# chongminggao/CIRS-codes

Measured on AMD Instinct MI355X. Metric: simulator env-steps/s (collect + PPO update in the timed region), KuaishouEnv, higher is better.
Workload: dtype f32 (policy/tracker; rollout on the fp32 MFMA, PPO head products fp32-accurate from two fp16 pieces per operand (3 f16 MFMAs per product), fp32 accumulate) + f64 (env rewards, GAE)

## Files before the change

### cirs-codes_amd/csrc/small_gemm.h

```cpp
#pragma once
#include "common.h"

namespace cirs {

typedef float sg_f32x16 __attribute__((ext_vector_type(16)));

template <bool kNT>
__device__ __forceinline__ void rows_gemm_body(int bx, int by, const float* __restrict__ X, int ldx, const float* __restrict__ W, int ldw,
                                               const float* __restrict__ bias, int R, int Kd, int N, int relu,
                                               const float* __restrict__ relu_of, int accumulate, float* __restrict__ Y, int ldy,
                                               const long* __restrict__ out_row) {
    const int lane = threadIdx.x, hi = lane >> 5, lo = lane & 31;
    const int row0 = bx * 32, n0 = by * 32;
    const int row = row0 + lo, n = n0 + lo;
    const bool row_ok = row < R, n_ok = n < N;
    sg_f32x16 acc;
    const float b = (bias && n_ok) ? bias[n] : 0.f;
#pragma unroll
    for (int s = 0; s < 16; ++s) acc[s] = b;
    const float* xr = X + (size_t)(row_ok ? row : 0) * ldx;
    if (kNT && (Kd & 31) == 0 && (ldx & 3) == 0 && ((uintptr_t)X & 15) == 0 && (ldw & 3) == 0 && ((uintptr_t)W & 15) == 0) {
        const float* wr = W + (size_t)(n_ok ? n : 0) * ldw;
        for (int kk = 0; kk < Kd; kk += 32) {
            float a[16], bv[16];
// ... 66 lines not shown
                                    const long* out_row = nullptr) {
    const dim3 grid(cdiv(R, 32), cdiv(N, 32));
    if (nt) hipLaunchKernelGGL(rows_gemm_kernel<true>, grid, dim3(64), 0, s, X, ldx, W, ldw, bias, R, Kd, N, relu, relu_of, accumulate, Y, ldy, out_row);
    else hipLaunchKernelGGL(rows_gemm_kernel<false>, grid, dim3(64), 0, s, X, ldx, W, ldw, bias, R, Kd, N, relu, relu_of, accumulate, Y, ldy, out_row);
}

constexpr int kDwMaxSlabs = 256;
__host__ inline int dwg_slabs(long R) {
    const long want = (R + 63) / 64;
    return (int)(want < 1 ? 1 : (want > kDwMaxSlabs ? kDwMaxSlabs : want));
}
__host__ inline size_t dwg_partial_floats(long R, int O, int K) { return (size_t)dwg_slabs(R) * O * (K + 1); }

__device__ __forceinline__ void dw_gemm_body(int bx, int slab, const float* __restrict__ dY, int ldy, const float* __restrict__ X, int ldx, int R,
                                             int O, int K, int rows_per_slab, float* __restrict__ partial) {
    const int lane = threadIdx.x, hi = lane >> 5, lo = lane & 31;
    const int k_tiles = (K + 31) / 32;
    const int o0 = (bx / k_tiles) * 32, k0 = (bx % k_tiles) * 32;
    const int r_beg = slab * rows_per_slab, r_end = min(R, r_beg + rows_per_slab);
    const int o = o0 + lo, k = k0 + lo;
    const bool o_ok = o < O, k_ok = k < K;
    sg_f32x16 acc;
#pragma unroll
    for (int s = 0; s < 16; ++s) acc[s] = 0.f;
    float bsum = 0.f;
    for (int r = r_beg; r < r_end; r += 64) {
        float a[32], b[32];
#pragma unroll
        for (int j = 0; j < 32; ++j) {
            const int rr = r + 2 * j + hi;
            const bool r_ok = rr < r_end;
// ... 185 lines not shown
```

### cirs-codes_amd/csrc/tracker_bwd.hip

```cpp
#include <algorithm>
#include "tracker_rows.h"
#include "rng.h"

namespace cirs {

#ifdef CIRS_TBWD_PROF
__device__ unsigned long long g_tbwd_prof[64];
#define CIRS_BSTAMP(K) do { if ((int)blockIdx.x == 300 && threadIdx.x == 0) g_tbwd_prof[K] = __builtin_amdgcn_s_memtime(); } while (0)
__device__ unsigned long long g_tbwd_wg[2048 * 3];
#define CIRS_BWG(SEL, WHICH) do { if ((SEL) && threadIdx.x == 0 && blockIdx.x < 2048) { g_tbwd_wg[blockIdx.x * 3 + (WHICH)] = __builtin_amdgcn_s_memtime(); \
    if ((WHICH) == 0) { unsigned hw; asm volatile("s_getreg_b32 %0, hwreg(HW_REG_HW_ID)" : "=s"(hw)); unsigned xcc; asm volatile("s_getreg_b32 %0, hwreg(HW_REG_XCC_ID)" : "=s"(xcc)); g_tbwd_wg[blockIdx.x * 3 + 2] = ((unsigned long long)xcc << 32) | hw; } } } while (0)
#else
#define CIRS_BSTAMP(K) do { } while (0)
#define CIRS_BWG(SEL, WHICH) do { } while (0)
#endif
constexpr int kChunkRows = 256;

struct DropCfg {
    int on;
    uint32_t thr;
    float inv;
    uint64_t seed;
    int env_base;
};
// ... 389 lines not shown
                }
            }
        }
#pragma unroll
        for (int h = 0; h < HPL; ++h) {
            const float ia = (kDrop ? dc.inv : 1.0f) / smA[h], ib = (kDrop ? dc.inv : 1.0f) / smB[h];
#pragma unroll
            for (int d = 0; d < HD; ++d) { accA[h * HD + d] *= ia; accB[h * HD + d] *= ib; }
        }
        if (actA) ep_store(ATT + (size_t)(base + pA) * tD + hg * DPL, accA, 1.0f);
        if (actB) ep_store(ATT + (size_t)(base + pB) * tD + hg * DPL, accB, 1.0f);
    }
}

template <int NH, bool kDrop>
__global__ __launch_bounds__(64) void attn_bwd_ep(const float* __restrict__ QKV, const float* __restrict__ dATT,
                                                  const int32_t* __restrict__ offsets, const int32_t* __restrict__ lens, int Lp,
                                                  float* __restrict__ dQKV, DropCfg dc, int layer,
                                                  const uint32_t* __restrict__ keep_in ) {
    using G = EpGeo<NH>;
    constexpr int HPL = G::HPL, DPL = G::DPL, HD = G::HD, SL = G::SL;
    extern __shared__ __attribute__((aligned(16))) float smem[];
    const int b = blockIdx.x, len = lens[b];
    if (len <= 0) return;
    const int lane = threadIdx.x, hg = lane / SL, slot = lane - hg * SL;
    const int base = offsets[b], STR = G::strip(Lp);
    float* sQKV = smem;
    float* sdA = smem + (size_t)Lp * 96;
    float* sS = sdA + (size_t)Lp * 32;
    float* sM = sS + (size_t)G::NW * (Lp + 1) * STR;
    float* sI = sM + (size_t)NH * Lp;
    uint32_t* sK = reinterpret_cast<uint32_t*>(sI + (size_t)NH * Lp);
    CIRS_BWG(layer == 1, 0);
    CIRS_BSTAMP(39);
    const int len32 = min(len, 32);
    f32x4 st_q[12], st_d[4];
    ep_stage_issue<96, 12>(st_q, QKV + (size_t)base * 96, len32, 96, lane);
    ep_stage_issue<tD, 4>(st_d, dATT + (size_t)base * tD, len32, tD, lane);
// ... 168 lines not shown
                }
            }
        }
        if (actA) {
            float* o = dQKV + (size_t)(base + jA) * 96 + 32 + hg * DPL;
            ep_store(o, dKA, scale); ep_store(o + 32, dVA, 1.0f);
        }
        if (actB) {
            float* o = dQKV + (size_t)(base + jB) * 96 + 32 + hg * DPL;
            ep_store(o, dKB, scale); ep_store(o + 32, dVB, 1.0f);
        }
    }
    CIRS_BSTAMP(42);
    CIRS_BWG(layer == 1, 1);
}
#undef EP_KEEP

constexpr int kRowT = 132;
__device__ __forceinline__ void mm_block(sg_f32x16& acc, const float (&a)[16], const float* __restrict__ wr) {
    float bv[16];
    ep_load(bv, wr);
#pragma unroll
    for (int j = 0; j < 16; ++j) acc = __builtin_amdgcn_mfma_f32_32x32x2f32(a[j], bv[j], acc, 0, 0, 0);
}
__device__ __forceinline__ void acc_to_lds(float* __restrict__ sT, const sg_f32x16& acc, int col, int hi) {
#pragma unroll
    for (int s = 0; s < 16; ++s) sT[acc_row(s, hi) * kRowT + col] = acc[s];
}
__device__ __forceinline__ void ln_half_row(const float (&y)[16], const float* __restrict__ g, const float* __restrict__ b, int hi,
                                            float (&xh)[16], float (&out)[16], float& rs) {
// ... 371 lines not shown
    acc_to_lds(sT, acc, lo, hi);
    __syncthreads();
    {
        float t[16];
        ep_load(t, sT + lo * kRowT + 16 * hi);
        if (row_ok) ep_store(a.dATT + rr * tD + 16 * hi, t, 1.0f);
    }
    CIRS_BSTAMP(28);
}

struct BwdScratch {
    float *G, *H[CIRS_MAX_TRACKER_LAYERS + 1];
    float *QKV[CIRS_MAX_TRACKER_LAYERS], *P[CIRS_MAX_TRACKER_LAYERS], *ATT[CIRS_MAX_TRACKER_LAYERS];
    float *XH1[CIRS_MAX_TRACKER_LAYERS], *RS1[CIRS_MAX_TRACKER_LAYERS], *H1N[CIRS_MAX_TRACKER_LAYERS], *FF1[CIRS_MAX_TRACKER_LAYERS];
    float *XH2[CIRS_MAX_TRACKER_LAYERS], *RS2[CIRS_MAX_TRACKER_LAYERS];
    float *T0, *T1, *T2, *T3, *T4, *T5, *dQKV, *dFF1, *dS, *partial, *GIN;
    float* LC;
    float* PM[CIRS_MAX_TRACKER_LAYERS];
    void* sort;
};

constexpr int kLastFloats = tD + 16 + 2 + 2;

static size_t bwd_partial_floats(const cirs_tracker_cfg* cfg, long R) {
    size_t f = dw_list_floats(R, 32, tD) + dw_list_floats(R, tD, tD) + dw_list_floats(R, tD, tD + 1);
    f += (size_t)cfg->nlayers * (2 * dw_list_floats(R, tD, tD) + dw_list_floats(R, tD, tH) + dw_list_floats(R, tH, tD) +
                                 dw_list_floats(R, tD, tD) + dw_list_floats(R, 96, tD));
    return f;
}

static size_t bwd_floats(const cirs_tracker_cfg* cfg, long R) {
    const long nl = cfg->nlayers, Lp = cfg->max_len, NH = cfg->nhead;
    size_t f = 0;
    f += (size_t)R * 32;
    f += (size_t)(nl + 1) * R * tD;
    f += (size_t)nl * R * (96 + NH * Lp + tD + tD + 1 + tD + tH + tD + 1);
    f += 6 * (size_t)R * tD + (size_t)R * 96 + (size_t)R * tH + (size_t)R * NH * Lp + 64;
    if (cfg->dropout_p > 0.f) f += (size_t)nl * R * NH * Lp + 64;
    f += bwd_partial_floats(cfg, R) + 4096;
    f += (size_t)R * (tD + 1);
    f += (size_t)R * kLastFloats;
    f += emb_sort_bytes(R + cfg->n_env) / 4 + 64;
    return f + 64 * 32;
}

static BwdScratch carve_bwd(void* ws, const cirs_tracker_cfg* cfg, long R) {
    float* p = (float*)ws;
    auto take = [&](size_t n) { float* r = p; p += (n + 3) & ~(size_t)3; return r; };
    const long nl = cfg->nlayers, Lp = cfg->max_len, NH = cfg->nhead;
    BwdScratch s;
    s.G = take((size_t)R * 32);
    for (int l = 0; l <= nl; ++l) s.H[l] = take((size_t)R * tD);
    for (int l = 0; l < nl; ++l) {
        s.QKV[l] = take((size_t)R * 96); s.P[l] = take((size_t)R * NH * Lp); s.ATT[l] = take((size_t)R * tD);
        s.XH1[l] = take((size_t)R * tD); s.RS1[l] = take(R); s.H1N[l] = take((size_t)R * tD); s.FF1[l] = take((size_t)R * tH);
        s.XH2[l] = take((size_t)R * tD); s.RS2[l] = take(R);
    }
    s.T0 = take((size_t)R * tD); s.T1 = take((size_t)R * tD); s.T2 = take((size_t)R * tD); s.T3 = take((size_t)R * tD);
    s.T4 = take((size_t)R * tD); s.T5 = take((size_t)R * tD);
    for (int l = 0; l < nl; ++l) s.PM[l] = cfg->dropout_p > 0.f ? take((size_t)R * NH * Lp) : nullptr;
    s.dQKV = take((size_t)R * 96); s.dFF1 = take((size_t)R * tH); s.dS = take((size_t)R * NH * Lp);
    s.partial = take(bwd_partial_floats(cfg, R) + 4096);
    s.GIN = take((size_t)R * (tD + 1));
    s.LC = take((size_t)R * kLastFloats);
    s.sort = (void*)take(emb_sort_bytes(R + cfg->n_env) / 4 + 64);
    return s;
}

}

#ifdef CIRS_TBWD_PROF
extern "C" int cirs_debug_tbwd_wg(unsigned long long* out_host) {
    return hipMemcpyFromSymbol(out_host, HIP_SYMBOL(cirs::g_tbwd_wg), 2048 * 3 * sizeof(unsigned long long)) == hipSuccess ? 0 : -2;
}
extern "C" int cirs_debug_tbwd_prof(unsigned long long* out_host64) {
    return hipMemcpyFromSymbol(out_host64, HIP_SYMBOL(cirs::g_tbwd_prof), 64 * sizeof(unsigned long long)) == hipSuccess ? 0 : -2;
// ... 617 lines not shown
    const bool ep = L <= 64 && ep_bytes(true) <= 64 * 1024 && !getenv("CIRS_TRACKER_ATTN_ROWS");
#define ATT_EP1(KERNEL, N, BWD, ...)                                                                                            \
    do {                                                                                                                        \
        if (dc.on) CIRS_LAUNCH_SPREAD((KERNEL<N, true>), B, 0, ep_bytes(BWD), s, __VA_ARGS__);       \
        else CIRS_LAUNCH_SPREAD((KERNEL<N, false>), B, 0, ep_bytes(BWD), s, __VA_ARGS__);           \
    } while (0)
#define ATT_EP(KERNEL, BWD, ...)                                  \
    do {                                                          \
        switch (NH) {                                             \
            case 1: ATT_EP1(KERNEL, 1, BWD, __VA_ARGS__); break;  \
            case 2: ATT_EP1(KERNEL, 2, BWD, __VA_ARGS__); break;  \
            case 4: ATT_EP1(KERNEL, 4, BWD, __VA_ARGS__); break;  \
            default: ATT_EP1(KERNEL, 8, BWD, __VA_ARGS__); break; \
        }                                                         \
    } while (0)

    DropCfg dc{};
    if (cfg->dropout_p > 0.f) {
        CIRS_REQUIRE(cfg->dropout_p < 1.f, "dropout_p must be in [0, 1)");
        dc.on = 1; dc.thr = dropout_threshold(cfg->dropout_p); dc.inv = 1.0f / (1.0f - cfg->dropout_p);
        dc.seed = cfg->dropout_seed; dc.env_base = cfg->drop_env_base;
    }
    if (state_out && ep && L <= 32 && S <= 64 && !getenv("CIRS_TRACKER_PREFIX_LAUNCHES")) {
        PrefixEnvArgs pa{};
        pa.x_hist = st->x_hist; pa.pe = w->pe; pa.row_env = row_env; pa.row_t = row_t; pa.offsets = offsets; pa.lens = lens;
        for (int l = 0; l < nl; ++l) pa.layer[l] = w->layer[l];
        pa.dec_w = w->dec_w; pa.dec_b = w->dec_b; pa.state_out = state_out; pa.state_stride = (long)state_stride; pa.nl = nl; pa.L = L; pa.S = S;
        if (ptf && ptf->on) {
            CIRS_REQUIRE(ptf->cfg.hidden == kH && ptf->cfg.dim_state == S && ptf->h2, "prefix states: trunk shape mismatch");
            pa.tf = *ptf;
// ... 64 lines not shown
        }
        LayerFwdArgs fa{sc.ATT[l], sc.H[l], y, l + 1 < nl ? w->layer[l + 1].in_proj_w : nullptr, l + 1 < nl ? w->layer[l + 1].in_proj_b : nullptr,
                        sc.XH1[l], sc.RS1[l], sc.H1N[l], sc.FF1[l], sc.XH2[l], sc.RS2[l], sc.H[l + 1], l + 1 < nl ? sc.QKV[l + 1] : nullptr,
                        row_env, row_t, R, l};
        if (dc.on) CIRS_LAUNCH_SPREAD(layer_rows_fwd<true>, cdiv(R, 32), 40 * 1024, 0, s, fa, dc);
        else CIRS_LAUNCH_SPREAD(layer_rows_fwd<false>, cdiv(R, 32), 40 * 1024, 0, s, fa, dc);
    }
    CIRS_CHECK_LAUNCH("tracker forward recompute");
    if (state_out) {
        hipLaunchKernelGGL(prefix_decoder_kernel, dim3(cdiv(B, 4)), dim3(256), 0, s, (const float*)sc.H[nl], lens, B, S, w->dec_w, w->dec_b,
                           state_out, (long)state_stride);
        CIRS_CHECK_LAUNCH("prefix_decoder_kernel");
        return CIRS_OK;
    }
    float* dH = sc.T0;
    if (top_last) {
        hipLaunchKernelGGL(dstate_last_rows, g1((long)B * S), dim3(256), 0, s, dstate_last, lens, B, S, sc.G);
        launch_rows_gemm(false, sc.G, S, w->dec_w, tD, nullptr, B, S, tD, 0, nullptr, 0, dH, tD, s);
    } else {
        if (dstate_last) hipLaunchKernelGGL(dstate_last_full, g1((long)R * S), dim3(256), 0, s, dstate_last, row_env, offsets, lens, R, S, sc.G);
        else hipLaunchKernelGGL(gather_dstate, g1((long)R * S), dim3(256), 0, s, dstate, row_env, row_t, R, S, B, sc.G);
        launch_rows_gemm_dw(dwl, sc.H[nl], tD, S, tD, grads->dec_w, grads->dec_b, sc.partial, false, sc.G, S, w->dec_w, tD, nullptr, R, S, tD, 0, nullptr, 0,
                            dH, tD, s);
    }
    for (int l = nl - 1; l >= 0; --l) {
        const cirs_tracker_layer& y = w->layer[l];
        const cirs_tracker_layer_grads& gy = grads->layer[l];
        if (top_last && l == nl - 1) {
            float* dB1 = dc.on ? sc.T4 : dY1c;
            LayerBwdArgs ba{sc.T0, nullptr, nullptr, nullptr, sc.T0, 0, y, sc.XH2[l], sc.RS2[l], sc.FF1[l], sc.XH1[l], sc.RS1[l], sc.T3, sc.dFF1, sc.T1, dY1c, dB1,
                            sc.T5, env_c, t_c, B, l};
            if (dc.on) CIRS_LAUNCH_SPREAD(layer_rows_bwd<true>, cdiv(B, 32), 40 * 1024, 0, s, ba, dc);
            else CIRS_LAUNCH_SPREAD(layer_rows_bwd<false>, cdiv(B, 32), 40 * 1024, 0, s, ba, dc);
            DwBatch bt{};
            dw_batch_add(bt, dwl, sc.G, S, sc.H[nl], tD, R, S, tD, grads->dec_w, grads->dec_b, 0, sc.partial);
            dw_batch_add(bt, dwl, sc.T0, tD, sc.XH2[l], tD, R, tD, tD, gy.norm2_w, gy.norm2_b, 1, sc.partial);
            dw_batch_add(bt, dwl, sc.T3, tD, sc.FF1[l], tH, R, tD, tH, gy.lin2_w, gy.lin2_b, 0, sc.partial);
            dw_batch_add(bt, dwl, sc.dFF1, tH, sc.H1N[l], tD, R, tH, tD, gy.lin1_w, gy.lin1_b, 0, sc.partial);
            dw_batch_add(bt, dwl, sc.T1, tD, sc.XH1[l], tD, R, tD, tD, gy.norm1_w, gy.norm1_b, 1, sc.partial);
            dw_batch_add(bt, dwl, dB1, tD, sc.ATT[l], tD, R, tD, tD, gy.out_proj_w, gy.out_proj_b, 0, sc.partial);
            dw_batch_launch(bt, R, s, B);
            ATT_LAST(attn_last_bwd, (const float*)sc.QKV[l], (const float*)sc.T5, (const float*)dY1c, (const float*)att_stats, offsets, lens, B, L, sc.dQKV,
                     sc.T2, dc, l);
            continue;
        }
        const bool pre = l + 1 < nl;
        float* dB1 = dc.on ? sc.T4 : sc.T2;
        LayerBwdArgs ba{sc.T0, pre ? sc.T2 : nullptr, pre ? sc.dQKV : nullptr, pre ? w->layer[l + 1].in_proj_w : nullptr, sc.T0, 0, y,
                        sc.XH2[l], sc.RS2[l], sc.FF1[l], sc.XH1[l], sc.RS1[l], sc.T3, sc.dFF1, sc.T1, sc.T2, dB1, sc.T5, row_env, row_t, R, l};
        if (dc.on) CIRS_LAUNCH_SPREAD(layer_rows_bwd<true>, cdiv(R, 32), 40 * 1024, 0, s, ba, dc);
        else CIRS_LAUNCH_SPREAD(layer_rows_bwd<false>, cdiv(R, 32), 40 * 1024, 0, s, ba, dc);
        DwBatch bt{};
        if (pre) dw_batch_add(bt, dwl, sc.dQKV, 96, sc.H[l + 1], tD, R, 96, tD, grads->layer[l + 1].in_proj_w, grads->layer[l + 1].in_proj_b, 0, sc.partial);
        dw_batch_add(bt, dwl, sc.T0, tD, sc.XH2[l], tD, R, tD, tD, gy.norm2_w, gy.norm2_b, 1, sc.partial);
        dw_batch_add(bt, dwl, sc.T3, tD, sc.FF1[l], tH, R, tD, tH, gy.lin2_w, gy.lin2_b, 0, sc.partial);
        dw_batch_add(bt, dwl, sc.dFF1, tH, sc.H1N[l], tD, R, tH, tD, gy.lin1_w, gy.lin1_b, 0, sc.partial);
        dw_batch_add(bt, dwl, sc.T1, tD, sc.XH1[l], tD, R, tD, tD, gy.norm1_w, gy.norm1_b, 1, sc.partial);
        dw_batch_add(bt, dwl, dB1, tD, sc.ATT[l], tD, R, tD, tD, gy.out_proj_w, gy.out_proj_b, 0, sc.partial);
        dw_batch_launch(bt, R, s);
        const float* dATT = sc.T5;
        if (ep) {
            ATT_EP(attn_bwd_ep, true, (const float*)sc.QKV[l], dATT, offsets, lens, L, sc.dQKV, dc, l, dc.on ? reinterpret_cast<const uint32_t*>(sc.P[l]) : (const uint32_t*)nullptr);
        } else {
            ATT_DISPATCH_SH(attn_bwd_q, (size_t)4 * NH * L * sizeof(float), sc.QKV[l], sc.P[l], dATT, row_env, row_t, offsets, R, L, sc.dS, sc.dQKV,
                            (const float*)sc.PM[l], dc.inv);
            ATT_DISPATCH(attn_bwd_kv, sc.QKV[l], dc.on ? sc.PM[l] : sc.P[l], sc.dS, dATT, row_env, row_t, offsets, lens, R, L, sc.dQKV);
        }
    }
    {
        LayerBwdArgs ba{};
        ba.dY1p = sc.T2; ba.dQKVp = sc.dQKV; ba.winp = w->layer[0].in_proj_w; ba.dHout = sc.T0; ba.only_pre = 1;
        ba.row_env = row_env; ba.row_t = row_t; ba.R = R;
        if (dc.on) CIRS_LAUNCH_SPREAD(layer_rows_bwd<true>, cdiv(R, 32), 40 * 1024, 0, s, ba, dc);
        else CIRS_LAUNCH_SPREAD(layer_rows_bwd<false>, cdiv(R, 32), 40 * 1024, 0, s, ba, dc);
    }
    CIRS_CHECK_LAUNCH("tracker backward layers");
    float* DU = sc.T1;
    float* EU = sc.H[nl];
    float* DPRE = sc.H1N[0];
    float* CU = sc.QKV[0];
    float* CI = sc.QKV[0] + (size_t)R * tD;
    int32_t* key_user = (int32_t*)sc.RS1[0];
    int32_t* key_item = (int32_t*)sc.RS2[0];
    const bool merged = B <= R;
    const int slot_rpw = R >= (1 << 17) ? 8 : 1;
    hipLaunchKernelGGL(slot_bwd, dim3(cdiv(R, 4 * slot_rpw)), dim3(256), 0, s, *w, dH, users, act, rew, row_env, row_t, R, B, DU, EU, DPRE,
                       sc.GIN, CU, CI, key_user, key_item, merged ? CI + (size_t)R * tD : nullptr, slot_rpw, 5.656854249492381f);
    if (merged) {
        if (int rc = emb_scatter_merged(key_item, users, lens, CI, R, B, cfg->n_items, cfg->n_users, grads->emb_item, grads->emb_user, sc.sort,
                                        emb_sort_bytes(R + B), s)) return rc;
    } else {
        int32_t* keys_c = (int32_t*)sc.T0;
        float* contrib_c = sc.T2;
        CIRS_HIP(hipMemsetAsync(keys_c, 0xFF, sizeof(int32_t) * (size_t)B, s));
        hipLaunchKernelGGL(compact_user_rows, dim3(cdiv(R, 8)), dim3(256), 0, s, row_env, row_t, users, (const float*)CU, R, keys_c, contrib_c);
        if (int rc = emb_scatter_sorted(keys_c, contrib_c, B, cfg->n_users, grads->emb_user, sc.sort, emb_sort_bytes(R), s)) return rc;
        if (int rc = emb_scatter_sorted(key_item, CI, R, cfg->n_items, grads->emb_item, sc.sort, emb_sort_bytes(R), s)) return rc;
    }
    DwBatch bt{};
    dw_batch_add(bt, dwl, sc.dQKV, 96, sc.H[0], tD, R, 96, tD, grads->layer[0].in_proj_w, grads->layer[0].in_proj_b, 0, sc.partial);
    dw_batch_add(bt, dwl, DU, tD, EU, tD, R, tD, tD, grads->ffn_user_w, grads->ffn_user_b, 0, sc.partial);
    dw_batch_add(bt, dwl, DPRE, tD, sc.GIN, tD + 1, R, tD, tD + 1, grads->gate_w, grads->gate_b, 0, sc.partial);
    dw_batch_launch(bt, R, s);
    launch_dw_list_final(dwl, R, sc.partial, s);
    CIRS_CHECK_LAUNCH("tracker backward slots");
#undef ATT_LAST
#undef ATT_LAST1
#undef ATT_DISPATCH
#undef ATT_EP
#undef ATT_EP1
#undef ATT_DISPATCH_SH
    return CIRS_OK;
}

extern "C" int cirs_tracker_backward(const cirs_tracker_cfg* cfg, const cirs_tracker_weights* w, const cirs_tracker_state* st,
                                     const int32_t* users, const int64_t* act, const double* rew, const int32_t* row_env,
                                     const int32_t* row_t, const int32_t* offsets, const int32_t* lens, int32_t n_rows,
                                     const float* dstate, const cirs_tracker_grads* grads, void* workspace,
                                     int64_t workspace_bytes, void* stream) {
    CIRS_REQUIRE(users && act && rew && dstate && grads, "null argument");
    return tracker_rows_impl(cfg, w, st, users, act, rew, row_env, row_t, offsets, lens, n_rows, dstate, grads, workspace, workspace_bytes, stream,
                             nullptr, 0);
}
// ... 42 lines not shown
```

### cirs-codes_amd/csrc/tracker_rows.h

```cpp
#pragma once
#include <hipcub/hipcub.hpp>
#include "small_gemm.h"
#include "internal.h"

namespace cirs {
typedef float f32x4 __attribute__((ext_vector_type(4)));

constexpr int tD = 32, tH = 128;

constexpr int kMaxDwBatch = 8;
struct DwBatchJob { const float* dY; int ldy; const float* X; int ldx; int O, K, tile_begin; float* partial; };
struct DwBatch { DwBatchJob j[kMaxDwBatch]; int n, total_tiles; };
static __global__ __launch_bounds__(64) void dw_batch_kernel(DwBatch jobs, int R, int rows_per_slab) {
    int ji = 0;
    for (; ji + 1 < jobs.n && (int)blockIdx.x >= jobs.j[ji + 1].tile_begin; ++ji) {}
    const DwBatchJob& jb = jobs.j[ji];
    dw_gemm_body((int)blockIdx.x - jb.tile_begin, blockIdx.y, jb.dY, jb.ldy, jb.X, jb.ldx, R, jb.O, jb.K, rows_per_slab, jb.partial);
}
static inline void dw_batch_add(DwBatch& b, DwList& list, const float* dY, int ldy, const float* X, int ldx, int R, int O, int K, float* dW,
                                float* db, int diag, float* partial) {
    const int slabs = dwg_slabs(R);
    DwListJob& lj = list.j[list.n++];
    lj.O = O; lj.K = K; lj.part_off = list.part_floats; lj.diag = diag; lj.dW = dW; lj.db = db;
    DwBatchJob& jb = b.j[b.n++];
    jb.dY = dY; jb.ldy = ldy; jb.X = X; jb.ldx = ldx; jb.O = O; jb.K = K; jb.tile_begin = b.total_tiles; jb.partial = partial + lj.part_off;
    b.total_tiles += cdiv(O, 32) * cdiv(K, 32);
    list.part_floats += slabs * O * (K + 1);
    list.total_out += O * (K + 1);
}
static inline void dw_batch_launch(const DwBatch& b, int R, hipStream_t s, int R_rows = -1) {
    if (!b.n) return;
    if (R_rows < 0) R_rows = R;
    const int slabs = dwg_slabs(R);
    int rows_per_slab = (R_rows + slabs - 1) / slabs;
    rows_per_slab = (rows_per_slab + 15) & ~15;
    hipLaunchKernelGGL(dw_batch_kernel, dim3(b.total_tiles, slabs), dim3(64), 0, s, b, R_rows, rows_per_slab);
}

static __global__ __launch_bounds__(256) void gather_dstate(const float* __restrict__ dstate, const int32_t* __restrict__ row_env,
                                                     const int32_t* __restrict__ row_t, int R, int S, int B, float* __restrict__ G) {
    const long i = blockIdx.x * (long)blockDim.x + threadIdx.x;
    if (i >= (long)R * S) return;
    const int r = (int)(i / S), s = (int)(i % S);
    G[i] = dstate[((size_t)row_t[r] * B + row_env[r]) * S + s];
}

__device__ __forceinline__ float lane_bcast(float x, int k) {
    return __builtin_bit_cast(float, __builtin_amdgcn_readlane(__builtin_bit_cast(int, x), k));
}

static __global__ __launch_bounds__(256) void slot_bwd(cirs_tracker_weights w, const float* __restrict__ dH0, const int32_t* __restrict__ users,
// ... 66 lines not shown
    rows[r] = r;
}

static __global__ __launch_bounds__(256) void compact_user_rows(const int32_t* __restrict__ row_env, const int32_t* __restrict__ row_t,
                                                         const int32_t* __restrict__ users, const float* __restrict__ CU, int R,
                                                         int32_t* __restrict__ keys_c, float* __restrict__ contrib_c) {
    const int d = threadIdx.x & 31;
    const int r = blockIdx.x * 8 + (threadIdx.x >> 5);
    if (r >= R || row_t[r] != 0) return;
    const int b = row_env[r];
    contrib_c[(size_t)b * tD + d] = CU[(size_t)r * tD + d];
    if (d == 0) keys_c[b] = users[b];
}

constexpr int kSubRun = 64;
static __global__ __launch_bounds__(256) void emb_subrun_kernel(const uint32_t* __restrict__ ks, const int32_t* __restrict__ rs,
                                                         const float* __restrict__ contrib, int R, int n_table, float* __restrict__ part) {
    const int d = threadIdx.x & 31, half = (threadIdx.x >> 5) & 1;
    const int p = blockIdx.x * 8 + (threadIdx.x >> 5);
    const bool in = p < R;
    const uint32_t key = in ? ks[p] : 0xffffffffu;
    const bool start = in && key < (uint32_t)n_table && ((p % kSubRun) == 0 || ks[p - 1] != key);
    const int end = min(R, (p / kSubRun + 1) * kSubRun);
    const int q0 = p + d, q1 = p + 32 + d;
    const bool s0 = start && q0 < end && ks[q0] == key, s1 = start && q1 < end && ks[q1] == key;
    const int r0 = s0 ? rs[q0] : 0, r1 = s1 ? rs[q1] : 0;
    const unsigned long long m0 = __ballot(s0), m1 = __ballot(s1);
    if (!start) return;
    const uint32_t h0 = (uint32_t)(m0 >> (32 * half)), h1 = (uint32_t)(m1 >> (32 * half));
    const int n = h0 == 0xffffffffu ? 32 + (h1 == 0xffffffffu ? 32 : __builtin_ctz(~h1)) : __builtin_ctz(~h0);
    float acc = 0.f;
    for (int q = 0; q < n; q += 16) {
        float t[16];
#pragma unroll
        for (int u = 0; u < 16; ++u) {
            const int qq = q + u;
            const int row = __shfl(qq < 32 ? r0 : r1, (qq & 31) + 32 * half, CIRS_WAVE);
            t[u] = qq < n ? contrib[(size_t)row * tD + d] : 0.f;
        }
#pragma unroll
        for (int u = 0; u < 16; ++u) acc += (q + u < n) ? t[u] : 0.f;
    }
    part[(size_t)p * tD + d] = acc;
}

static __global__ __launch_bounds__(256) void emb_segment_sum_kernel(const uint32_t* __restrict__ ks, const float* __restrict__ part, int R,
                                                              int n_table, float* __restrict__ g_emb, int n_first = 0x7fffffff,
                                                              float* __restrict__ g_second = nullptr) {
    const int d = threadIdx.x & 31;
    const int p = blockIdx.x * 8 + (threadIdx.x >> 5);
    if (p >= R) return;
    const uint32_t key = ks[p];
    if (key >= (uint32_t)n_table || (p > 0 && ks[p - 1] == key)) return;
    float acc = part[(size_t)p * tD + d];
    for (int q = (p / kSubRun + 1) * kSubRun; q < R; q += 8 * kSubRun) {
        float t8[8];
        int n_ok = 0;
#pragma unroll
// ... 28 lines not shown
    size_t need = 0;
    CIRS_HIP(hipcub::DeviceRadixSort::SortPairs(nullptr, need, k_in, k_out, r_in, r_out, R, 0, end_bit, s));
    CIRS_REQUIRE(need <= avail, "embedding scatter: sort scratch too small");
    CIRS_HIP(hipMemsetAsync(g_emb, 0, (size_t)n_table * tD * sizeof(float), s));
    hipLaunchKernelGGL(scatter_keys_kernel, dim3(cdiv(R, 256)), dim3(256), 0, s, keys, R, n_table, k_in, r_in);
    CIRS_HIP(hipcub::DeviceRadixSort::SortPairs(temp, need, k_in, k_out, r_in, r_out, R, 0, end_bit, s));
    hipLaunchKernelGGL(emb_subrun_kernel, dim3(cdiv(R, 8)), dim3(256), 0, s, k_out, r_out, contrib, R, n_table, part);
    hipLaunchKernelGGL(emb_segment_sum_kernel, dim3(cdiv(R, 8)), dim3(256), 0, s, k_out, (const float*)part, R, n_table, g_emb);
    CIRS_CHECK_LAUNCH("emb_segment_sum_kernel");
    return CIRS_OK;
}

static __global__ __launch_bounds__(256) void scatter_keys2_kernel(const int32_t* __restrict__ key_item, const int32_t* __restrict__ users,
                                                            const int32_t* __restrict__ lens, int R, int B, int n_items, int n_users,
                                                            uint32_t* __restrict__ keys_u, int32_t* __restrict__ rows,
                                                            float* __restrict__ zero_table , long zero_floats) {
    const int p = blockIdx.x * blockDim.x + threadIdx.x;
    if (zero_table)
        for (long i = (long)p * 4; i < zero_floats; i += (long)gridDim.x * blockDim.x * 4) *reinterpret_cast<f32x4*>(zero_table + i) = f32x4{0.f, 0.f, 0.f, 0.f};
    if (p >= R + B) return;
    const uint32_t sent = (uint32_t)n_items + (uint32_t)n_users;
    uint32_t k = sent;
    if (p < R) {
        const int32_t v = key_item[p];
        if (v >= 0 && v < n_items) k = (uint32_t)v;
    } else {
        const int b = p - R;
        const int32_t u = users[b];
        if (lens[b] > 0 && u >= 0 && u < n_users) k = (uint32_t)n_items + (uint32_t)u;
    }
    keys_u[p] = k;
    rows[p] = p;
}
static int emb_scatter_merged(const int32_t* key_item, const int32_t* users, const int32_t* lens, const float* contrib, int R, int B,
                              int n_items, int n_users, float* g_item, float* g_user, void* scratch, size_t scratch_bytes, hipStream_t s) {
    const int N = R + B, n_table = n_items + n_users;
    uint32_t* k_in = (uint32_t*)scratch;
    uint32_t* k_out = k_in + N;
    int32_t* r_in = (int32_t*)(k_out + N);
    int32_t* r_out = r_in + N;
    float* part = (float*)(((uintptr_t)(r_out + N) + 255) & ~(uintptr_t)255);
    char* temp = (char*)(((uintptr_t)(part + (size_t)N * tD) + 255) & ~(uintptr_t)255);
    const size_t avail = scratch_bytes - (size_t)(temp - (char*)scratch);
    int end_bit = 1;
    while ((1u << end_bit) <= (uint32_t)n_table && end_bit < 32) ++end_bit;
    size_t need = 0;
    CIRS_HIP(hipcub::DeviceRadixSort::SortPairs(nullptr, need, k_in, k_out, r_in, r_out, N, 0, end_bit, s));
    CIRS_REQUIRE(need <= avail, "embedding scatter: sort scratch too small");
    float* zero_table = nullptr;
    if (g_user + (size_t)n_users * tD == g_item) zero_table = g_user;
    else if (g_item + (size_t)n_items * tD == g_user) zero_table = g_item;
    if (zero_table && ((uintptr_t)zero_table & 15)) zero_table = nullptr;
    if (!zero_table) {
        CIRS_HIP(hipMemsetAsync(g_item, 0, (size_t)n_items * tD * sizeof(float), s));
        CIRS_HIP(hipMemsetAsync(g_user, 0, (size_t)n_users * tD * sizeof(float), s));
    }
    hipLaunchKernelGGL(scatter_keys2_kernel, dim3(cdiv(N, 256)), dim3(256), 0, s, key_item, users, lens, R, B, n_items, n_users, k_in, r_in, zero_table,
                       (long)n_table * tD);
    CIRS_HIP(hipcub::DeviceRadixSort::SortPairs(temp, need, k_in, k_out, r_in, r_out, N, 0, end_bit, s));
    hipLaunchKernelGGL(emb_subrun_kernel, dim3(cdiv(N, 8)), dim3(256), 0, s, k_out, r_out, contrib, N, n_table, part);
    hipLaunchKernelGGL(emb_segment_sum_kernel, dim3(cdiv(N, 8)), dim3(256), 0, s, k_out, (const float*)part, N, n_table, g_item, n_items, g_user);
    CIRS_CHECK_LAUNCH("emb_segment_sum_kernel (merged)");
    return CIRS_OK;
}

}
```

Measured before the change: 5.976 million.

## Co-launch weight-gradient GEMMs with attention backward and embedding subrun kernels

Merges the batched weight-gradient GEMM tiles into the same launch as the per-sequence attention backward kernel (when the combined grid fits on the CUs) and into the embedding subrun kernel. This lets independent work share one grid instead of running as separate serialized launches. dQKV is double-buffered across layers so the next layer's dW can read the previous buffer while attention writes the other. Separate item/user gradient-table memsets are also folded into the key scatter kernel. The cost is extra scratch memory, 256-thread blocks where most lanes idle for the attention role, and possible LDS and occupancy interactions.

Result: no change. 5.977 million (median of 3 runs) (+0.0%).

```diff
diff --git a/cirs-codes_amd/csrc/small_gemm.h b/cirs-codes_amd/csrc/small_gemm.h
--- a/cirs-codes_amd/csrc/small_gemm.h
+++ b/cirs-codes_amd/csrc/small_gemm.h
@@ -104,7 +104,7 @@
 
 __device__ __forceinline__ void dw_gemm_body(int bx, int slab, const float* __restrict__ dY, int ldy, const float* __restrict__ X, int ldx, int R,
                                              int O, int K, int rows_per_slab, float* __restrict__ partial) {
-    const int lane = threadIdx.x, hi = lane >> 5, lo = lane & 31;
+    const int lane = threadIdx.x & 63, hi = lane >> 5, lo = lane & 31;
     const int k_tiles = (K + 31) / 32;
     const int o0 = (bx / k_tiles) * 32, k0 = (bx % k_tiles) * 32;
     const int r_beg = slab * rows_per_slab, r_end = min(R, r_beg + rows_per_slab);
diff --git a/cirs-codes_amd/csrc/tracker_bwd.hip b/cirs-codes_amd/csrc/tracker_bwd.hip
--- a/cirs-codes_amd/csrc/tracker_bwd.hip
+++ b/cirs-codes_amd/csrc/tracker_bwd.hip
@@ -427,14 +427,14 @@
 }
 
 template <int NH, bool kDrop>
-__global__ __launch_bounds__(64) void attn_bwd_ep(const float* __restrict__ QKV, const float* __restrict__ dATT,
-                                                  const int32_t* __restrict__ offsets, const int32_t* __restrict__ lens, int Lp,
-                                                  float* __restrict__ dQKV, DropCfg dc, int layer,
-                                                  const uint32_t* __restrict__ keep_in ) {
+__device__ __forceinline__ void attn_bwd_ep_body(int b, const float* __restrict__ QKV, const float* __restrict__ dATT,
+                                                 const int32_t* __restrict__ offsets, const int32_t* __restrict__ lens, int Lp,
+                                                 float* __restrict__ dQKV, const DropCfg& dc, int layer,
+                                                 const uint32_t* __restrict__ keep_in ) {
     using G = EpGeo<NH>;
     constexpr int HPL = G::HPL, DPL = G::DPL, HD = G::HD, SL = G::SL;
     extern __shared__ __attribute__((aligned(16))) float smem[];
-    const int b = blockIdx.x, len = lens[b];
+    const int len = lens[b];
     if (len <= 0) return;
     const int lane = threadIdx.x, hg = lane / SL, slot = lane - hg * SL;
     const int base = offsets[b], STR = G::strip(Lp);
@@ -633,6 +633,24 @@
     CIRS_BSTAMP(42);
     CIRS_BWG(layer == 1, 1);
 }
+template <int NH, bool kDrop>
+__global__ __launch_bounds__(64) void attn_bwd_ep(const float* __restrict__ QKV, const float* __restrict__ dATT,
+                                                  const int32_t* __restrict__ offsets, const int32_t* __restrict__ lens, int Lp,
+                                                  float* __restrict__ dQKV, DropCfg dc, int layer, const uint32_t* __restrict__ keep_in) {
+    attn_bwd_ep_body<NH, kDrop>((int)blockIdx.x, QKV, dATT, offsets, lens, Lp, dQKV, dc, layer, keep_in);
+}
+template <int NH, bool kDrop>
+__global__ __launch_bounds__(256) void attn_bwd_ep_dw(const float* __restrict__ QKV, const float* __restrict__ dATT,
+                                                      const int32_t* __restrict__ offsets, const int32_t* __restrict__ lens, int Lp,
+                                                      float* __restrict__ dQKV, DropCfg dc, int layer, const uint32_t* __restrict__ keep_in,
+                                                      int n_ep, DwBatchRole dw) {
+    if ((int)blockIdx.x < n_ep) {
+        if (threadIdx.x >= 64) return;
+        attn_bwd_ep_body<NH, kDrop>((int)blockIdx.x, QKV, dATT, offsets, lens, Lp, dQKV, dc, layer, keep_in);
+    } else {
+        dw_batch_role(dw, (int)blockIdx.x - n_ep);
+    }
+}
 #undef EP_KEEP
 
 constexpr int kRowT = 132;
@@ -1034,7 +1052,7 @@
     float *QKV[CIRS_MAX_TRACKER_LAYERS], *P[CIRS_MAX_TRACKER_LAYERS], *ATT[CIRS_MAX_TRACKER_LAYERS];
     float *XH1[CIRS_MAX_TRACKER_LAYERS], *RS1[CIRS_MAX_TRACKER_LAYERS], *H1N[CIRS_MAX_TRACKER_LAYERS], *FF1[CIRS_MAX_TRACKER_LAYERS];
     float *XH2[CIRS_MAX_TRACKER_LAYERS], *RS2[CIRS_MAX_TRACKER_LAYERS];
-    float *T0, *T1, *T2, *T3, *T4, *T5, *dQKV, *dFF1, *dS, *partial, *GIN;
+    float *T0, *T1, *T2, *T3, *T4, *T5, *dQKV, *dQKV2, *dFF1, *dS, *partial, *GIN;
     float* LC;
     float* PM[CIRS_MAX_TRACKER_LAYERS];
     void* sort;
@@ -1055,7 +1073,7 @@
     f += (size_t)R * 32;
     f += (size_t)(nl + 1) * R * tD;
     f += (size_t)nl * R * (96 + NH * Lp + tD + tD + 1 + tD + tH + tD + 1);
-    f += 6 * (size_t)R * tD + (size_t)R * 96 + (size_t)R * tH + (size_t)R * NH * Lp + 64;
+    f += 6 * (size_t)R * tD + 2 * (size_t)R * 96 + (size_t)R * tH + (size_t)R * NH * Lp + 64;
     if (cfg->dropout_p > 0.f) f += (size_t)nl * R * NH * Lp + 64;
     f += bwd_partial_floats(cfg, R) + 4096;
     f += (size_t)R * (tD + 1);
@@ -1079,7 +1097,7 @@
     s.T0 = take((size_t)R * tD); s.T1 = take((size_t)R * tD); s.T2 = take((size_t)R * tD); s.T3 = take((size_t)R * tD);
     s.T4 = take((size_t)R * tD); s.T5 = take((size_t)R * tD);
     for (int l = 0; l < nl; ++l) s.PM[l] = cfg->dropout_p > 0.f ? take((size_t)R * NH * Lp) : nullptr;
-    s.dQKV = take((size_t)R * 96); s.dFF1 = take((size_t)R * tH); s.dS = take((size_t)R * NH * Lp);
+    s.dQKV = take((size_t)R * 96); s.dQKV2 = take((size_t)R * 96); s.dFF1 = take((size_t)R * tH); s.dS = take((size_t)R * NH * Lp);
     s.partial = take(bwd_partial_floats(cfg, R) + 4096);
     s.GIN = take((size_t)R * (tD + 1));
     s.LC = take((size_t)R * kLastFloats);
@@ -1727,6 +1745,22 @@
             default: ATT_EP1(KERNEL, 8, BWD, __VA_ARGS__); break; \
         }                                                         \
     } while (0)
+#define ATT_EP_DW1(N, DROP, ROLE, ...)                                                                                          \
+    do {                                                                                                                        \
+        const size_t dyn_ = spread_dyn_lds((long)B, 0, ep_bytes(true));                                                         \
+        if (dyn_ != ep_bytes(true)) lds_optin(attn_bwd_ep_dw<N, DROP>, dyn_);                                                   \
+        hipLaunchKernelGGL((attn_bwd_ep_dw<N, DROP>), dim3(B + dw_batch_role_groups(ROLE)), dim3(256), dyn_, s, __VA_ARGS__, B, ROLE); \
+    } while (0)
+#define ATT_EP_DW(ROLE, ...)                                                                                                   \
+    do {                                                                                                                       \
+        switch (NH) {                                                                                                          \
+            case 1: if (dc.on) ATT_EP_DW1(1, true, ROLE, __VA_ARGS__); else ATT_EP_DW1(1, false, ROLE, __VA_ARGS__); break;    \
+            case 2: if (dc.on) ATT_EP_DW1(2, true, ROLE, __VA_ARGS__); else ATT_EP_DW1(2, false, ROLE, __VA_ARGS__); break;    \
+            case 4: if (dc.on) ATT_EP_DW1(4, true, ROLE, __VA_ARGS__); else ATT_EP_DW1(4, false, ROLE, __VA_ARGS__); break;    \
+            default: if (dc.on) ATT_EP_DW1(8, true, ROLE, __VA_ARGS__); else ATT_EP_DW1(8, false, ROLE, __VA_ARGS__); break;   \
+        }                                                                                                                      \
+    } while (0)
+    const bool separate = getenv("CIRS_TRACKER_BWD_SEPARATE") != nullptr;
 
     DropCfg dc{};
     if (cfg->dropout_p > 0.f) {
@@ -1821,6 +1855,7 @@
         return CIRS_OK;
     }
     float* dH = sc.T0;
+    auto dqkv = [&](int l) { return (l & 1) ? sc.dQKV2 : sc.dQKV; };
     if (top_last) {
         hipLaunchKernelGGL(dstate_last_rows, g1((long)B * S), dim3(256), 0, s, dstate_last, lens, B, S, sc.G);
         launch_rows_gemm(false, sc.G, S, w->dec_w, tD, nullptr, B, S, tD, 0, nullptr, 0, dH, tD, s);
@@ -1847,36 +1882,42 @@
             dw_batch_add(bt, dwl, sc.T1, tD, sc.XH1[l], tD, R, tD, tD, gy.norm1_w, gy.norm1_b, 1, sc.partial);
             dw_batch_add(bt, dwl, dB1, tD, sc.ATT[l], tD, R, tD, tD, gy.out_proj_w, gy.out_proj_b, 0, sc.partial);
             dw_batch_launch(bt, R, s, B);
-            ATT_LAST(attn_last_bwd, (const float*)sc.QKV[l], (const float*)sc.T5, (const float*)dY1c, (const float*)att_stats, offsets, lens, B, L, sc.dQKV,
+            ATT_LAST(attn_last_bwd, (const float*)sc.QKV[l], (const float*)sc.T5, (const float*)dY1c, (const float*)att_stats, offsets, lens, B, L, dqkv(l),
                      sc.T2, dc, l);
             continue;
         }
         const bool pre = l + 1 < nl;
         float* dB1 = dc.on ? sc.T4 : sc.T2;
-        LayerBwdArgs ba{sc.T0, pre ? sc.T2 : nullptr, pre ? sc.dQKV : nullptr, pre ? w->layer[l + 1].in_proj_w : nullptr, sc.T0, 0, y,
+        LayerBwdArgs ba{sc.T0, pre ? sc.T2 : nullptr, pre ? dqkv(l + 1) : nullptr, pre ? w->layer[l + 1].in_proj_w : nullptr, sc.T0, 0, y,
                         sc.XH2[l], sc.RS2[l], sc.FF1[l], sc.XH1[l], sc.RS1[l], sc.T3, sc.dFF1, sc.T1, sc.T2, dB1, sc.T5, row_env, row_t, R, l};
         if (dc.on) CIRS_LAUNCH_SPREAD(layer_rows_bwd<true>, cdiv(R, 32), 40 * 1024, 0, s, ba, dc);
         else CIRS_LAUNCH_SPREAD(layer_rows_bwd<false>, cdiv(R, 32), 40 * 1024, 0, s, ba, dc);
         DwBatch bt{};
-        if (pre) dw_batch_add(bt, dwl, sc.dQKV, 96, sc.H[l + 1], tD, R, 96, tD, grads->layer[l + 1].in_proj_w, grads->layer[l + 1].in_proj_b, 0, sc.partial);
+        if (pre) dw_batch_add(bt, dwl, dqkv(l + 1), 96, sc.H[l + 1], tD, R, 96, tD, grads->layer[l + 1].in_proj_w, grads->layer[l + 1].in_proj_b, 0, sc.partial);
         dw_batch_add(bt, dwl, sc.T0, tD, sc.XH2[l], tD, R, tD, tD, gy.norm2_w, gy.norm2_b, 1, sc.partial);
         dw_batch_add(bt, dwl, sc.T3, tD, sc.FF1[l], tH, R, tD, tH, gy.lin2_w, gy.lin2_b, 0, sc.partial);
         dw_batch_add(bt, dwl, sc.dFF1, tH, sc.H1N[l], tD, R, tH, tD, gy.lin1_w, gy.lin1_b, 0, sc.partial);
         dw_batch_add(bt, dwl, sc.T1, tD, sc.XH1[l], tD, R, tD, tD, gy.norm1_w, gy.norm1_b, 1, sc.partial);
         dw_batch_add(bt, dwl, dB1, tD, sc.ATT[l], tD, R, tD, tD, gy.out_proj_w, gy.out_proj_b, 0, sc.partial);
+        const float* dATT = sc.T5;
+        const uint32_t* keep_in = dc.on ? reinterpret_cast<const uint32_t*>(sc.P[l]) : (const uint32_t*)nullptr;
+        const DwBatchRole role = dw_batch_role_of(bt, R);
+        if (ep && !separate && B + dw_batch_role_groups(role) <= device_cu_count()) {
+            ATT_EP_DW(role, (const float*)sc.QKV[l], dATT, offsets, lens, L, dqkv(l), dc, l, keep_in);
+            continue;
+        }
         dw_batch_launch(bt, R, s);
-        const float* dATT = sc.T5;
         if (ep) {
-            ATT_EP(attn_bwd_ep, true, (const float*)sc.QKV[l], dATT, offsets, lens, L, sc.dQKV, dc, l, dc.on ? reinterpret_cast<const uint32_t*>(sc.P[l]) : (const uint32_t*)nullptr);
+            ATT_EP(attn_bwd_ep, true, (const float*)sc.QKV[l], dATT, offsets, lens, L, dqkv(l), dc, l, keep_in);
         } else {
-            ATT_DISPATCH_SH(attn_bwd_q, (size_t)4 * NH * L * sizeof(float), sc.QKV[l], sc.P[l], dATT, row_env, row_t, offsets, R, L, sc.dS, sc.dQKV,
+            ATT_DISPATCH_SH(attn_bwd_q, (size_t)4 * NH * L * sizeof(float), sc.QKV[l], sc.P[l], dATT, row_env, row_t, offsets, R, L, sc.dS, dqkv(l),
                             (const float*)sc.PM[l], dc.inv);
-            ATT_DISPATCH(attn_bwd_kv, sc.QKV[l], dc.on ? sc.PM[l] : sc.P[l], sc.dS, dATT, row_env, row_t, offsets, lens, R, L, sc.dQKV);
+            ATT_DISPATCH(attn_bwd_kv, sc.QKV[l], dc.on ? sc.PM[l] : sc.P[l], sc.dS, dATT, row_env, row_t, offsets, lens, R, L, dqkv(l));
         }
     }
     {
         LayerBwdArgs ba{};
-        ba.dY1p = sc.T2; ba.dQKVp = sc.dQKV; ba.winp = w->layer[0].in_proj_w; ba.dHout = sc.T0; ba.only_pre = 1;
+        ba.dY1p = sc.T2; ba.dQKVp = dqkv(0); ba.winp = w->layer[0].in_proj_w; ba.dHout = sc.T0; ba.only_pre = 1;
         ba.row_env = row_env; ba.row_t = row_t; ba.R = R;
         if (dc.on) CIRS_LAUNCH_SPREAD(layer_rows_bwd<true>, cdiv(R, 32), 40 * 1024, 0, s, ba, dc);
         else CIRS_LAUNCH_SPREAD(layer_rows_bwd<false>, cdiv(R, 32), 40 * 1024, 0, s, ba, dc);
@@ -1893,9 +1934,15 @@
     const int slot_rpw = R >= (1 << 17) ? 8 : 1;
     hipLaunchKernelGGL(slot_bwd, dim3(cdiv(R, 4 * slot_rpw)), dim3(256), 0, s, *w, dH, users, act, rew, row_env, row_t, R, B, DU, EU, DPRE,
                        sc.GIN, CU, CI, key_user, key_item, merged ? CI + (size_t)R * tD : nullptr, slot_rpw, 5.656854249492381f);
+    DwBatch bt{};
+    dw_batch_add(bt, dwl, dqkv(0), 96, sc.H[0], tD, R, 96, tD, grads->layer[0].in_proj_w, grads->layer[0].in_proj_b, 0, sc.partial);
+    dw_batch_add(bt, dwl, DU, tD, EU, tD, R, tD, tD, grads->ffn_user_w, grads->ffn_user_b, 0, sc.partial);
+    dw_batch_add(bt, dwl, DPRE, tD, sc.GIN, tD + 1, R, tD, tD + 1, grads->gate_w, grads->gate_b, 0, sc.partial);
+    const bool ride = merged && !separate;
     if (merged) {
+        const DwBatchRole role = dw_batch_role_of(bt, R);
         if (int rc = emb_scatter_merged(key_item, users, lens, CI, R, B, cfg->n_items, cfg->n_users, grads->emb_item, grads->emb_user, sc.sort,
-                                        emb_sort_bytes(R + B), s)) return rc;
+                                        emb_sort_bytes(R + B), s, ride ? &role : nullptr, !separate)) return rc;
     } else {
         int32_t* keys_c = (int32_t*)sc.T0;
         float* contrib_c = sc.T2;
@@ -1904,16 +1951,14 @@
         if (int rc = emb_scatter_sorted(keys_c, contrib_c, B, cfg->n_users, grads->emb_user, sc.sort, emb_sort_bytes(R), s)) return rc;
         if (int rc = emb_scatter_sorted(key_item, CI, R, cfg->n_items, grads->emb_item, sc.sort, emb_sort_bytes(R), s)) return rc;
     }
-    DwBatch bt{};
-    dw_batch_add(bt, dwl, sc.dQKV, 96, sc.H[0], tD, R, 96, tD, grads->layer[0].in_proj_w, grads->layer[0].in_proj_b, 0, sc.partial);
-    dw_batch_add(bt, dwl, DU, tD, EU, tD, R, tD, tD, grads->ffn_user_w, grads->ffn_user_b, 0, sc.partial);
-    dw_batch_add(bt, dwl, DPRE, tD, sc.GIN, tD + 1, R, tD, tD + 1, grads->gate_w, grads->gate_b, 0, sc.partial);
-    dw_batch_launch(bt, R, s);
+    if (!ride) dw_batch_launch(bt, R, s);
     launch_dw_list_final(dwl, R, sc.partial, s);
     CIRS_CHECK_LAUNCH("tracker backward slots");
 #undef ATT_LAST
 #undef ATT_LAST1
 #undef ATT_DISPATCH
+#undef ATT_EP_DW
+#undef ATT_EP_DW1
 #undef ATT_EP
 #undef ATT_EP1
 #undef ATT_DISPATCH_SH
diff --git a/cirs-codes_amd/csrc/tracker_rows.h b/cirs-codes_amd/csrc/tracker_rows.h
--- a/cirs-codes_amd/csrc/tracker_rows.h
+++ b/cirs-codes_amd/csrc/tracker_rows.h
@@ -11,11 +11,20 @@
 constexpr int kMaxDwBatch = 8;
 struct DwBatchJob { const float* dY; int ldy; const float* X; int ldx; int O, K, tile_begin; float* partial; };
 struct DwBatch { DwBatchJob j[kMaxDwBatch]; int n, total_tiles; };
+__device__ __forceinline__ void dw_batch_body(const DwBatch& jobs, int tile, int slab, int R, int rows_per_slab) {
+    int ji = 0;
+    for (; ji + 1 < jobs.n && tile >= jobs.j[ji + 1].tile_begin; ++ji) {}
+    const DwBatchJob& jb = jobs.j[ji];
+    dw_gemm_body(tile - jb.tile_begin, slab, jb.dY, jb.ldy, jb.X, jb.ldx, R, jb.O, jb.K, rows_per_slab, jb.partial);
+}
 static __global__ __launch_bounds__(64) void dw_batch_kernel(DwBatch jobs, int R, int rows_per_slab) {
-    int ji = 0;
-    for (; ji + 1 < jobs.n && (int)blockIdx.x >= jobs.j[ji + 1].tile_begin; ++ji) {}
-    const DwBatchJob& jb = jobs.j[ji];
-    dw_gemm_body((int)blockIdx.x - jb.tile_begin, blockIdx.y, jb.dY, jb.ldy, jb.X, jb.ldx, R, jb.O, jb.K, rows_per_slab, jb.partial);
+    dw_batch_body(jobs, (int)blockIdx.x, (int)blockIdx.y, R, rows_per_slab);
+}
+struct DwBatchRole { DwBatch jobs; int R_rows, rows_per_slab, slabs; };
+__device__ __forceinline__ void dw_batch_role(const DwBatchRole& r, int group) {
+    const int unit = group * 4 + __builtin_amdgcn_readfirstlane((int)(threadIdx.x >> 6));
+    if (unit >= r.jobs.total_tiles * r.slabs) return;
+    dw_batch_body(r.jobs, unit % r.jobs.total_tiles, unit / r.jobs.total_tiles, r.R_rows, r.rows_per_slab);
 }
 static inline void dw_batch_add(DwBatch& b, DwList& list, const float* dY, int ldy, const float* X, int ldx, int R, int O, int K, float* dW,
                                 float* db, int diag, float* partial) {
@@ -28,13 +37,18 @@
     list.part_floats += slabs * O * (K + 1);
     list.total_out += O * (K + 1);
 }
-static inline void dw_batch_launch(const DwBatch& b, int R, hipStream_t s, int R_rows = -1) {
-    if (!b.n) return;
+static inline DwBatchRole dw_batch_role_of(const DwBatch& b, int R, int R_rows = -1) {
     if (R_rows < 0) R_rows = R;
     const int slabs = dwg_slabs(R);
     int rows_per_slab = (R_rows + slabs - 1) / slabs;
     rows_per_slab = (rows_per_slab + 15) & ~15;
-    hipLaunchKernelGGL(dw_batch_kernel, dim3(b.total_tiles, slabs), dim3(64), 0, s, b, R_rows, rows_per_slab);
+    return DwBatchRole{b, R_rows, rows_per_slab, slabs};
+}
+static inline int dw_batch_role_groups(const DwBatchRole& r) { return cdiv(r.jobs.total_tiles * r.slabs, 4); }
+static inline void dw_batch_launch(const DwBatch& b, int R, hipStream_t s, int R_rows = -1) {
+    if (!b.n) return;
+    const DwBatchRole r = dw_batch_role_of(b, R, R_rows);
+    hipLaunchKernelGGL(dw_batch_kernel, dim3(b.total_tiles, r.slabs), dim3(64), 0, s, b, r.R_rows, r.rows_per_slab);
 }
 
 static __global__ __launch_bounds__(256) void gather_dstate(const float* __restrict__ dstate, const int32_t* __restrict__ row_env,
@@ -131,10 +145,10 @@
 }
 
 constexpr int kSubRun = 64;
-static __global__ __launch_bounds__(256) void emb_subrun_kernel(const uint32_t* __restrict__ ks, const int32_t* __restrict__ rs,
-                                                         const float* __restrict__ contrib, int R, int n_table, float* __restrict__ part) {
+__device__ __forceinline__ void emb_subrun_body(int blk, const uint32_t* __restrict__ ks, const int32_t* __restrict__ rs,
+                                                const float* __restrict__ contrib, int R, int n_table, float* __restrict__ part) {
     const int d = threadIdx.x & 31, half = (threadIdx.x >> 5) & 1;
-    const int p = blockIdx.x * 8 + (threadIdx.x >> 5);
+    const int p = blk * 8 + (threadIdx.x >> 5);
     const bool in = p < R;
     const uint32_t key = in ? ks[p] : 0xffffffffu;
     const bool start = in && key < (uint32_t)n_table && ((p % kSubRun) == 0 || ks[p - 1] != key);
@@ -159,6 +173,16 @@
         for (int u = 0; u < 16; ++u) acc += (q + u < n) ? t[u] : 0.f;
     }
     part[(size_t)p * tD + d] = acc;
+}
+static __global__ __launch_bounds__(256) void emb_subrun_kernel(const uint32_t* __restrict__ ks, const int32_t* __restrict__ rs,
+                                                         const float* __restrict__ contrib, int R, int n_table, float* __restrict__ part) {
+    emb_subrun_body((int)blockIdx.x, ks, rs, contrib, R, n_table, part);
+}
+static __global__ __launch_bounds__(256) void emb_subrun_dw_kernel(const uint32_t* __restrict__ ks, const int32_t* __restrict__ rs,
+                                                            const float* __restrict__ contrib, int R, int n_table, float* __restrict__ part,
+                                                            int n_dw, DwBatchRole dw) {
+    if ((int)blockIdx.x < n_dw) dw_batch_role(dw, (int)blockIdx.x);
+    else emb_subrun_body((int)blockIdx.x - n_dw, ks, rs, contrib, R, n_table, part);
 }
 
 static __global__ __launch_bounds__(256) void emb_segment_sum_kernel(const uint32_t* __restrict__ ks, const float* __restrict__ part, int R,
@@ -217,10 +241,14 @@
 static __global__ __launch_bounds__(256) void scatter_keys2_kernel(const int32_t* __restrict__ key_item, const int32_t* __restrict__ users,
                                                             const int32_t* __restrict__ lens, int R, int B, int n_items, int n_users,
                                                             uint32_t* __restrict__ keys_u, int32_t* __restrict__ rows,
-                                                            float* __restrict__ zero_table , long zero_floats) {
+                                                            float* __restrict__ zero_table ,
+                                                            long zero_floats, float* __restrict__ zero_second ,
+                                                            long second_floats) {
     const int p = blockIdx.x * blockDim.x + threadIdx.x;
     if (zero_table)
         for (long i = (long)p * 4; i < zero_floats; i += (long)gridDim.x * blockDim.x * 4) *reinterpret_cast<f32x4*>(zero_table + i) = f32x4{0.f, 0.f, 0.f, 0.f};
+    if (zero_second)
+        for (long i = (long)p * 4; i < second_floats; i += (long)gridDim.x * blockDim.x * 4) *reinterpret_cast<f32x4*>(zero_second + i) = f32x4{0.f, 0.f, 0.f, 0.f};
     if (p >= R + B) return;
     const uint32_t sent = (uint32_t)n_items + (uint32_t)n_users;
     uint32_t k = sent;
@@ -236,7 +264,8 @@
     rows[p] = p;
 }
 static int emb_scatter_merged(const int32_t* key_item, const int32_t* users, const int32_t* lens, const float* contrib, int R, int B,
-                              int n_items, int n_users, float* g_item, float* g_user, void* scratch, size_t scratch_bytes, hipStream_t s) {
+                              int n_items, int n_users, float* g_item, float* g_user, void* scratch, size_t scratch_bytes, hipStream_t s,
+                              const DwBatchRole* ride = nullptr, bool fold_clears = true) {
     const int N = R + B, n_table = n_items + n_users;
     uint32_t* k_in = (uint32_t*)scratch;
     uint32_t* k_out = k_in + N;
@@ -254,14 +283,25 @@
     if (g_user + (size_t)n_users * tD == g_item) zero_table = g_user;
     else if (g_item + (size_t)n_items * tD == g_user) zero_table = g_item;
     if (zero_table && ((uintptr_t)zero_table & 15)) zero_table = nullptr;
+    long zero_floats = (long)n_table * tD, second_floats = 0;
+    float* zero_second = nullptr;
+    if (!zero_table && fold_clears && !((uintptr_t)g_item & 15) && !((uintptr_t)g_user & 15)) {
+        zero_table = g_item; zero_floats = (long)n_items * tD;
+        zero_second = g_user; second_floats = (long)n_users * tD;
+    }
     if (!zero_table) {
         CIRS_HIP(hipMemsetAsync(g_item, 0, (size_t)n_items * tD * sizeof(float), s));
         CIRS_HIP(hipMemsetAsync(g_user, 0, (size_t)n_users * tD * sizeof(float), s));
     }
     hipLaunchKernelGGL(scatter_keys2_kernel, dim3(cdiv(N, 256)), dim3(256), 0, s, key_item, users, lens, R, B, n_items, n_users, k_in, r_in, zero_table,
-                       (long)n_table * tD);
+                       zero_floats, zero_second, second_floats);
     CIRS_HIP(hipcub::DeviceRadixSort::SortPairs(temp, need, k_in, k_out, r_in, r_out, N, 0, end_bit, s));
-    hipLaunchKernelGGL(emb_subrun_kernel, dim3(cdiv(N, 8)), dim3(256), 0, s, k_out, r_out, contrib, N, n_table, part);
+    if (ride && ride->jobs.n) {
+        const int n_dw = dw_batch_role_groups(*ride);
+        hipLaunchKernelGGL(emb_subrun_dw_kernel, dim3(n_dw + cdiv(N, 8)), dim3(256), 0, s, k_out, r_out, contrib, N, n_table, part, n_dw, *ride);
+    } else {
+        hipLaunchKernelGGL(emb_subrun_kernel, dim3(cdiv(N, 8)), dim3(256), 0, s, k_out, r_out, contrib, N, n_table, part);
+    }
     hipLaunchKernelGGL(emb_segment_sum_kernel, dim3(cdiv(N, 8)), dim3(256), 0, s, k_out, (const float*)part, N, n_table, g_item, n_items, g_user);
     CIRS_CHECK_LAUNCH("emb_segment_sum_kernel (merged)");
     return CIRS_OK;
```
